# Tony-Tseng/deep-rawburst-sr

Hardware: AMD Instinct MI355X
Metric: bursts/sec 14x48x48 RAW->4x (SyntheticBurstVal shape), DBSR forward (higher is better)
Workload: dtype fp16; 1 GPU; configs[1]: SyntheticBurstVal 14-frame 48x48 -> 384x384 (sr x8 of RAW, x4 of full-res), batch 8 per GPU, full PWC-Net + warp + fusion + decoder; global_batch=8, frames=14, height=48, width=48, out_size=384, parallelism=dp1 (independent bursts per rank), hip_graph=True, fusion_weights_written=True

## Files before the change

deep-rawburst-sr_amd/_lib.py:

```python
import ctypes
import os

import torch

_HERE = os.path.dirname(os.path.abspath(__file__))
LIB_PATH = os.environ.get('DBSR_HIP_LIB', os.path.join(_HERE, 'libdbsr_hip.so'))

DBSR_F32, DBSR_BF16, DBSR_F16 = 0, 1, 2
ACT_NONE, ACT_RELU, ACT_LRELU = 0, 1, 2
OUT_NHWC, OUT_SHUFFLE, OUT_NCHW_F32 = 0, 1, 2
ABI_VERSION = 23
SRC_F32_NCHW, SRC_U8_NHWC = 0, 1
POST_GAINS, POST_CCM, POST_GAMMA, POST_SMOOTHSTEP = 1, 2, 4, 8


class FrameMap(ctypes.Structure):
    _fields_ = [('fpg', ctypes.c_int), ('group_stride', ctypes.c_int), ('group_offset', ctypes.c_int),
                ('inner_stride', ctypes.c_int)]


IDENTITY = (1, 1, 0, 1)


class Tensor(ctypes.Structure):
# ... 39 lines not shown
_lib = None


class DBSRLibError(RuntimeError):
    pass


def lib():
    global _lib
    if _lib is None:
        if not os.path.exists(LIB_PATH):
            raise DBSRLibError('libdbsr_hip.so not found at %s: build it with `make` (or __graft_entry__.build())'
                               % LIB_PATH)
        L = ctypes.CDLL(LIB_PATH)
        c_int, c_void_p, c_float, c_ll, c_size_t = (ctypes.c_int, ctypes.c_void_p, ctypes.c_float,
                                                    ctypes.c_longlong, ctypes.c_size_t)
        sigs = {
            'dbsr_abi_version': ([], c_int),
            'dbsr_last_error': ([], ctypes.c_char_p),
            'dbsr_conv_packed_elems': ([c_int, c_int, c_int, c_int], c_size_t),
            'dbsr_weights_round_diffuse': ([c_void_p, c_int, c_int, c_int, c_int, c_int, c_void_p, c_void_p], c_int),
            'dbsr_conv_pack_weights': ([c_void_p, c_void_p, c_int, c_int, c_int, c_int, c_int, c_int, c_void_p,
                                        c_void_p, c_void_p], c_int),
            'dbsr_pack_batch_prepare': ([ctypes.POINTER(PackJob), c_int], c_ll),
            'dbsr_conv_pack_weights_batch': ([c_void_p, c_int, c_ll, c_void_p], c_int),
            'dbsr_conv2d': ([ctypes.POINTER(ConvDesc), c_void_p], c_int),
            'dbsr_set_conv_algo': ([c_int], c_int),
            'dbsr_conv_kernel_for': ([ctypes.POINTER(ConvDesc)], c_int),
            'dbsr_conv_dispatch_variant': ([ctypes.POINTER(ConvDesc)], c_int),
            'dbsr_conv_lane_reach': ([ctypes.POINTER(ConvDesc), c_int], c_int),
            'dbsr_conv_workspace_bytes': ([ctypes.POINTER(ConvDesc)], c_size_t),
            'dbsr_conv2d_head': ([ctypes.POINTER(ConvDesc), c_void_p, c_void_p, c_int, Tensor, c_void_p], c_int),
            'dbsr_conv_head_ok': ([ctypes.POINTER(ConvDesc)], c_int),
            'dbsr_conv_shuffle_blur': ([ctypes.POINTER(ConvDesc), c_void_p, c_void_p], c_int),
            'dbsr_conv_shuffle_blur_ok': ([ctypes.POINTER(ConvDesc)], c_int),
            'dbsr_resblock': ([ctypes.POINTER(ConvDesc), ctypes.POINTER(ConvDesc), c_void_p], c_int),
            'dbsr_resblock_ok': ([ctypes.POINTER(ConvDesc), ctypes.POINTER(ConvDesc)], c_int),
            'dbsr_resblock_head': ([ctypes.POINTER(ConvDesc), ctypes.POINTER(ConvDesc), c_void_p, c_void_p, c_int, Tensor,
                                    c_void_p], c_int),
            'dbsr_correlation': ([c_int, c_int, c_int, c_int, Tensor, Tensor, Tensor, c_int, c_void_p], c_int),
            'dbsr_correlation_backward': ([c_int, c_int, c_int, c_int, Tensor, Tensor, Tensor, Tensor, c_int, Tensor,
                                           Tensor, c_void_p], c_int),
            'dbsr_backwarp': ([c_int, c_int, c_int, c_int, Tensor, Tensor, c_float, Tensor, c_void_p], c_int),
            'dbsr_warp_bilinear': ([c_int, c_int, c_int, c_int, Tensor, c_void_p, c_ll, Tensor, c_void_p], c_int),
            'dbsr_warp_project': ([c_int, c_int, c_int, c_int, Tensor, c_void_p, c_ll, Tensor, c_void_p, c_void_p, c_int,
                                   Tensor, c_void_p], c_int),
            'dbsr_fuse_relu_norm': ([c_int, c_int, c_int, c_int, Tensor, Tensor, Tensor, Tensor, Tensor, c_void_p], c_int),
            'dbsr_burst_mean': ([c_int, c_int, c_int, c_int, Tensor, Tensor, c_void_p], c_int),
            'dbsr_fuse_softmax': ([c_int, c_int, c_int, c_int, Tensor, Tensor, Tensor, Tensor, Tensor, c_void_p],
                                  c_int),
            'dbsr_conv_fuse_softmax': ([ctypes.POINTER(ConvDesc), c_int, c_int, Tensor, Tensor, Tensor, Tensor,
                                        c_void_p], c_int),
            'dbsr_conv_fuse_relu_norm': ([ctypes.POINTER(ConvDesc), c_int, c_int, Tensor, Tensor, Tensor, Tensor,
                                          c_void_p], c_int),
            'dbsr_conv_fuse_ok': ([ctypes.POINTER(ConvDesc), c_int, c_int], c_int),
            'dbsr_fuse_partial': ([c_int, c_int, c_int, c_int, c_int, Tensor, Tensor, Tensor, c_void_p, c_void_p], c_int),
            'dbsr_fuse_combine': ([c_int, c_int, c_int, c_int, c_void_p, Tensor, c_void_p], c_int),
            'dbsr_conv_transpose_k4s2': ([c_int, c_int, c_int, c_int, c_int, Tensor, c_void_p, c_void_p, Tensor,
                                          c_void_p], c_int),
            'dbsr_pack_burst': ([c_int, c_int, c_int, c_int, c_void_p, Tensor, c_int, c_int, Tensor, c_void_p], c_int),
            'dbsr_flow_finalize': ([c_int, c_int, c_int, c_int, Tensor, c_int, c_int, c_int, c_int, c_void_p, c_float,
                                    Tensor, c_void_p], c_int),
            'dbsr_gauss_blur3': ([c_int, c_int, c_int, c_int, Tensor, c_void_p, Tensor, c_void_p], c_int),
            'dbsr_merge_prep': ([c_int, c_int, c_int, c_int, Tensor, Tensor, c_void_p], c_int),
            'dbsr_pwc_assemble': ([c_int, c_int, c_int, c_int, Tensor, Tensor, Tensor, Tensor, c_void_p], c_int),
            'dbsr_zero': ([c_void_p, c_size_t, c_void_p], c_int),
# ... 56 lines not shown
            'dbsr_burst_synth': ([c_int, c_int, c_int, c_int, c_int, c_int, c_void_p, c_void_p, c_void_p, c_void_p,
                                  c_void_p, c_void_p, c_void_p, c_void_p], c_int),
            'dbsr_postprocess_rgb': ([c_int, c_int, c_int, c_void_p, c_void_p, c_int, c_void_p, c_void_p, c_void_p],
                                     c_int),
        }
        for name, (args, res) in sigs.items():
            fn = getattr(L, name)
            fn.argtypes = args
            fn.restype = res
        if L.dbsr_abi_version() != ABI_VERSION:
            raise DBSRLibError('libdbsr_hip.so ABI %d != expected %d' % (L.dbsr_abi_version(), ABI_VERSION))
        _lib = L
    return _lib


EXPORTED = ['dbsr_abi_version', 'dbsr_last_error', 'dbsr_conv_packed_elems', 'dbsr_conv_pack_weights',
            'dbsr_pack_batch_prepare', 'dbsr_conv_pack_weights_batch',
            'dbsr_weights_round_diffuse', 'dbsr_fuse_relu_norm', 'dbsr_burst_mean', 'dbsr_conv2d',
            'dbsr_set_conv_algo', 'dbsr_conv_kernel_for', 'dbsr_conv_dispatch_variant', 'dbsr_conv_lane_reach', 'dbsr_conv_workspace_bytes', 'dbsr_conv2d_head',
            'dbsr_conv_head_ok', 'dbsr_conv_shuffle_blur', 'dbsr_conv_shuffle_blur_ok', 'dbsr_resblock', 'dbsr_resblock_ok', 'dbsr_resblock_head',
            'dbsr_correlation', 'dbsr_correlation_backward', 'dbsr_backwarp', 'dbsr_warp_bilinear', 'dbsr_warp_project', 'dbsr_fuse_softmax',
            'dbsr_fuse_partial', 'dbsr_fuse_combine', 'dbsr_conv_fuse_softmax', 'dbsr_conv_fuse_relu_norm', 'dbsr_conv_fuse_ok',
            'dbsr_conv_transpose_k4s2', 'dbsr_pack_burst', 'dbsr_flow_finalize', 'dbsr_gauss_blur3',
            'dbsr_merge_prep', 'dbsr_pwc_assemble', 'dbsr_zero', 'dbsr_nhwc_to_nchw_f32', 'dbsr_conv_wgrad_workspace_bytes', 'dbsr_conv_wgrad', 'dbsr_conv_wgrad_bias', 'dbsr_set_wgrad_algo', 'dbsr_head_forward', 'dbsr_head_backward_workspace_bytes', 'dbsr_head_backward',
            'dbsr_chan_sum_workspace_bytes', 'dbsr_chan_sum', 'dbsr_l1_loss_backward', 'dbsr_relu_grad', 'dbsr_unshuffle_gate',
            'dbsr_fuse_backward', 'dbsr_merge_prep_backward', 'dbsr_warp_backward', 'dbsr_enc_grad_gate',
            'dbsr_warp_backward_gather_workspace_bytes', 'dbsr_warp_backward_gather', 'dbsr_gate_copy',
            'dbsr_adam_step', 'dbsr_dgrad_weights',
            'dbsr_resize_bilinear', 'dbsr_gauss_reflect', 'dbsr_color_fit', 'dbsr_color_apply', 'dbsr_pwc_dense',
            'dbsr_pwc_dense_supported', 'dbsr_pwc_refine', 'dbsr_pwc_refine_supported', 'dbsr_pwc_extract',
            'dbsr_pwc_extract_supported', 'dbsr_pwc_level_prep', 'dbsr_pwc_level_prep_supported',
            'dbsr_aligned_l1_workspace_bytes', 'dbsr_aligned_l1_forward', 'dbsr_aligned_l1_backward',
            'dbsr_ssim_workspace_bytes', 'dbsr_ssim_forward', 'dbsr_ssim_backward',
            'dbsr_unprocess_rgb', 'dbsr_burst_synth', 'dbsr_postprocess_rgb']


def check(rc, what):
    if rc != 0:
        msg = lib().dbsr_last_error().decode(errors='replace')
        raise DBSRLibError('%s failed (rc=%d): %s' % (what, rc, msg))


def dtype_code(dt):
    if dt == torch.float32:
        return DBSR_F32
    if dt == torch.bfloat16:
        return DBSR_BF16
    if dt == torch.float16:
        return DBSR_F16
    raise ValueError('unsupported dtype %s' % dt)


def tensor_desc(t, ld, c0=0, img_stride=None, fmap=IDENTITY, dtype=None):
    if t is None:
        return Tensor(None, 0, 0, 0, 0, FrameMap(1, 1, 0, 1))
    if img_stride is None:
        img_stride = t[0].numel() if t.dim() > 1 else t.numel()
    return Tensor(t.data_ptr(), dtype_code(t.dtype if dtype is None else dtype), int(img_stride), int(ld), int(c0),
                  FrameMap(*fmap))


NULL_TENSOR = Tensor(None, 0, 0, 0, 0, FrameMap(1, 1, 0, 1))


def stream_ptr(device=None):
    return torch.cuda.current_stream(device).cuda_stream
```

deep-rawburst-sr_amd/engine.py:

```python
import ctypes
import math
import os
import types

import torch

from . import _lib as L
from ._lib import IDENTITY

BACKWARP_SCALE = {5: 0.625, 4: 1.25, 3: 2.5, 2: 5.0}
PWC_LEVEL_CH = {1: 16, 2: 32, 3: 64, 4: 96, 5: 128, 6: 196}
DENSE_OUT = [128, 128, 96, 64, 32]
DENSE_OFF = [320, 192, 96, 32, 0]
BASE_OFF = 448
REFINER_TAIL = [(128, 128, 3, 2), (128, 128, 3, 4), (128, 96, 3, 8), (96, 64, 3, 16), (64, 32, 3, 1), (32, 2, 3, 1)]


def r8(c):
    return (c + 7) // 8 * 8


def cpad(c):
    return r8(c) if c <= 16 else (c + 31) // 32 * 32

# ... 169 lines not shown
        return st

    def switch(self, lane):
        assert lane == 0 or lane in self.streams or not Plan.MULTI_STREAM
        self.lane = lane if Plan.MULTI_STREAM else 0

    def join(self, lane):
        if not Plan.MULTI_STREAM:
            return
        assert lane != 0 and lane in self.streams
        self.ops.append((Plan.JOIN, (torch.cuda.Event(),), f'sync.join{lane}', lane))
        self.lane = 0

    def conv(self, name, pc, n_frames, x, xc0, in_hw, y, yc0, act, xmap=IDENTITY, ymap=IDENTITY, res=None,
             rc0=0, rmap=IDENTITY, post_act=L.ACT_NONE, out_mode=L.OUT_NHWC, shuffle=0, y_desc=None, cin=None,
             precise=False, head=None, gate=None, gc0=0, gmap=IDENTITY):
        d = self._desc(name, pc, n_frames, x, xc0, in_hw, y, yc0, act, xmap, ymap, res, rc0, rmap, post_act,
                       out_mode, shuffle, y_desc, cin, precise, gate, gc0, gmap)
        self.convs.append((d, self.lane))
        oh, ow = d.out_h, d.out_w
        flop = 2.0 * n_frames * oh * ow * pc.cout * d.cin * pc.kh * pc.kw
        d.fused_head = bool(head is not None and L.lib().dbsr_conv_head_ok(ctypes.byref(d)))
        if d.fused_head:
            hname, hw, hb, hdesc = head
            self.keep.extend([hw, hb, hdesc])
            flop += 2.0 * n_frames * oh * ow * hw.shape[0] * hw.shape[1]
            self.add(name + '+' + hname, L.lib().dbsr_conv2d_head, ctypes.byref(d), hw.data_ptr(),
                     hb.data_ptr() if hb is not None else None, hw.shape[0], hdesc, work=('flop', flop))
            self.kernel[len(self.ops) - 1] = 'conv3x3_pipe'
            return d
        self.add(name, L.lib().dbsr_conv2d, ctypes.byref(d), work=('flop', flop))
        self.kernel[len(self.ops) - 1] = {4: 'conv3x3_ws', 7: 'conv3x3_ks128', 2: 'conv3x3_pipe', 1: 'conv3x3_tiled', 3: 'conv1x1_shuffle', 5: 'conv1x1', 6: 'conv3x3_narrow', 8: 'conv3x3_small'}.get(L.lib().dbsr_conv_kernel_for(d),
                                                                                      'conv2d_generic')
        return d

    def conv_fuse(self, name, pc, B, N, x, in_hw, ref, oth, fused, weights, xmap=IDENTITY, softmax=True):
        d = self._desc(name, pc, B * N, x, 0, in_hw, None, 0, L.ACT_NONE, xmap, IDENTITY, None, 0, IDENTITY,
                       L.ACT_NONE, L.OUT_NHWC, 0, L.NULL_TENSOR, None, False, None, 0, IDENTITY)
        if not L.lib().dbsr_conv_fuse_ok(ctypes.byref(d), B, N):
            return None
        H, W = in_hw
        flop = 2.0 * B * N * H * W * pc.cout * d.cin * pc.kh * pc.kw
        fn = L.lib().dbsr_conv_fuse_softmax if softmax else L.lib().dbsr_conv_fuse_relu_norm
        self.add(name, fn, ctypes.byref(d), B, N, ref, oth, fused, weights,
                 work=('flop', flop))
        self.kernel[len(self.ops) - 1] = 'conv_fuse'
        es, C = (4 if x.dtype == torch.float32 else 2), pc.cout
        self.hbm[len(self.ops) - 1] = es * B * H * W * (N * d.cin + N * C + (N * C if weights.ptr else 0) + C)
        return len(self.ops) - 1

    def resblock(self, name, c1, c2, n_frames, x, mid, y, hw, head=None, yc0=0):
        d1 = self._desc(name + '.conv1', c1, n_frames, x, 0, hw, mid, 0, L.ACT_RELU, IDENTITY, IDENTITY, None, 0,
                        IDENTITY, L.ACT_NONE, L.OUT_NHWC, 0, None, None, False, None, 0, IDENTITY)
        d2 = self._desc(name + '.conv2', c2, n_frames, mid, 0, hw, y, yc0, L.ACT_NONE, IDENTITY, IDENTITY, x, 0,
                        IDENTITY, L.ACT_RELU, L.OUT_NHWC, 0, None, None, False, None, 0, IDENTITY)
        if (c1.cout == 64 and not DBSREngine.FUSED_RESBLOCK64) or \
                not L.lib().dbsr_resblock_ok(ctypes.byref(d1), ctypes.byref(d2)):
            return False
        self.convs.extend([(d1, self.lane), (d2, self.lane)])
        oh, ow = d1.out_h, d1.out_w
        flop = 2.0 * n_frames * oh * ow * (c1.cout * d1.cin * 9 + c2.cout * d2.cin * 9)
        if head is not None:
            hname, hw_, hb, hdesc = head
            self.keep.extend([hw_, hb, hdesc])
            flop += 2.0 * n_frames * oh * ow * hw_.shape[0] * hw_.shape[1]
            self.add(name + '+' + hname, L.lib().dbsr_resblock_head, ctypes.byref(d1), ctypes.byref(d2),
# ... 261 lines not shown
                    plan.add(f'pwc.dec{level}.upflow', lib.dbsr_conv_transpose_k4s2, P, pD.h, pD.w, 2, 2, pflow.d(0),
                             wt.data_ptr(), bs.data_ptr(), fu.d(0))
                    wt, bs = ent['upfeat']
                    plan.add(f'pwc.dec{level}.upfeat', lib.dbsr_conv_transpose_k4s2, P, pD.h, pD.w, BASE_OFF + pbase,
                             2, pD.d(0), wt.data_ptr(), bs.data_ptr(), fe.d(0))
                    ws = NHWC(P, h, w, cpad(C), dtype, device)
                    plan.add(f'pwc.dec{level}.backwarp', lib.dbsr_backwarp, P, h, w, C, feat.d(0, second_map), fu.d(0),
                             BACKWARP_SCALE[level], ws.d(0))
                    plan.add(f'pwc.dec{level}.assemble', lib.dbsr_pwc_assemble, P, h, w, C, feat.d(0, first_map),
                             fu.d(0), fe.d(0), D.d(BASE_OFF))
                    second = ws.d(0)
                    plan.keep.extend([fu, fe, ws])
                plan.add(f'pwc.dec{level}.corr', lib.dbsr_correlation, P, h, w, C, feat.d(0, first_map), second,
                         D.d(BASE_OFF), 1)
            fl = NHWC(P, h, w, 8, torch.float32, device)
            if PWCPlanner.FUSED_DENSE and dtype != torch.float32 and lib.dbsr_pwc_dense_supported(h, w, ld):
                convs = (L.PwcDenseConv * 6)()
                cin, flop = base_real, 0.0
                for i, pc in enumerate(ent['dense'] + [ent['flow']]):
                    start = 0 if i == 5 else (BASE_OFF if i == 0 else DENSE_OFF[i - 1])
                    cg = cpad(pc.cin) // 8
                    convs[i] = L.PwcDenseConv(pc.w.data_ptr(), pc.bias.data_ptr() if pc.bias is not None else None,
                                              9 * cg * 8, cg, start, pc.cout, DENSE_OFF[i] if i < 5 else 0)
                    flop += 2.0 * P * h * w * pc.cout * pc.cin * 9
                plan.keep.append(convs)
                plan.add(f'pwc.dec{level}.dense', lib.dbsr_pwc_dense, P, h, w, D.d(0), BASE_OFF, convs, fl.d(0),
                         work=('flop', flop))
                plan.kernel[len(plan.ops) - 1] = 'pwc_dense'
                cin = base_real + sum(DENSE_OUT)
            else:
                cin = base_real
                for i, (pc, off) in enumerate(zip(ent['dense'], DENSE_OFF)):
                    start = BASE_OFF if i == 0 else DENSE_OFF[i - 1]
                    plan.conv(f'pwc.dec{level}.dense{i}', pc, P, D, start, (h, w), D, off, L.ACT_LRELU, cin=cin)
                    cin += DENSE_OUT[i]
                plan.conv(f'pwc.dec{level}.flow', ent['flow'], P, D, 0, (h, w), None, 0, L.ACT_NONE, cin=cin,
                          y_desc=fl.d(0))
            plan.keep.extend([D, fl])
            prev = (D, fl, base_real)
        D2, fl2, base2 = prev
        h, w = D2.h, D2.w
        chans = [128, 128, 128, 96, 64, 32]
        bufs = [NHWC(P, h, w, cpad(c), dtype, device) for c in chans]
        x, xc0, cin = D2, 0, BASE_OFF + base2
        fused = PWCPlanner.FUSED_REFINER and dtype != torch.float32 and \
            lib.dbsr_pwc_refine_supported(h, w, L.dtype_code(dtype)) and \
            [(pc.cin, pc.cout, pc.kh, pc.dil) for pc in self.ref[1:]] == REFINER_TAIL
        for i in range(1 if fused else 6):
            pc = self.ref[i]
            if pc.dil >= h and pc.dil >= w and pc.kh == 3:
                pc = self.ref_center(i)
            plan.conv(f'pwc.refiner{i}', pc, P, x, xc0, (h, w), bufs[i], 0, L.ACT_LRELU, cin=cin)
            x, xc0, cin = bufs[i], 0, chans[i]
        if fused:
            pcs = [self.ref_center(i) if i == 4 else self.ref[i] for i in range(1, 7)]
            convs = (L.PwcRefineConv * 6)(*[
                L.PwcRefineConv(pc.w.data_ptr(), pc.bias.data_ptr() if pc.bias is not None else None, pc.cin, pc.cout,
                                pc.kh, pc.dil) for pc in pcs])
            flop = sum(2.0 * P * h * w * pc.cout * pc.cin * pc.kh * pc.kw for pc in pcs)
            plan.keep.append(convs)
            plan.add('pwc.refiner1-6', lib.dbsr_pwc_refine, P, h, w, x.d(0), convs, fl2.d(0), flow_out.d(0),
                     work=('flop', flop))
            plan.kernel[len(plan.ops) - 1] = 'pwc_dense'
        else:
            plan.conv('pwc.refiner6', self.ref[6], P, x, 0, (h, w), None, 0, L.ACT_NONE, y_desc=flow_out.d(0),
                      res=fl2)
        plan.keep.extend(bufs)


class DBSREngine:
    LANE0_CU_SHARE = 0.5625
    LANE0_EARLY_CONVS = 0
    LANE0_EARLY_SHARE = 0.5
    FUSED_HEAD = True
    FUSED_UPSAMPLE_BLUR = True
    FUSED_RESBLOCK = True
    FUSED_RESBLOCK64 = True
    FUSED_WARP_PROJ = False
    LINEAR_SPLIT = True
    FUSED_WP_OUT = True
    WEIGHT_ROUNDING = 'diffuse'

    def __init__(self, net):
        self.net = net
        self.dtype = net.compute_dtype
        self.zero_flow = bool(getattr(net, 'zero_flow', False))
        self.device = None
        self.sig = None
        self.plans = {}
        self.slots = {}
        self.graphs = {}
        self.weights_stale = False

    def matches(self, net):
        return (net is self.net and self.dtype == net.compute_dtype and self.sig == _param_signature(net)
                and self.zero_flow == bool(getattr(net, 'zero_flow', False)))

    def _pack(self, device):
        net = self.net
        stream = L.stream_ptr(device)
        W = _Weights(self.dtype, device, stream, rounding=DBSREngine.WEIGHT_ROUNDING)
        enc, mer, dec = net.encoder, net.merging, net.decoder
        self.pwc = PWCPlanner(enc.alignment_net, _Weights(self.dtype, device, stream))
        self.enc_init = W.conv(enc.init_layer[0])
        self.enc_res = [(W.conv(b.conv1[0]), W.conv(b.conv2[0])) for b in enc.res_layers]
        self.enc_out = W.conv(enc.out_layer[0])
        self.proj = W.conv(mer.feat_project_layer[0])
        ofe = list(mer.offset_feat_extractor)
        self.ofe_init = W.conv(ofe[0][0])
        self.ofe_res = [(W.conv(b.conv1[0]), W.conv(b.conv2[0])) for b in ofe[1:]]
        wp = list(mer.weight_predictor)
        self.wp_init = W.conv(wp[0][0])
        self.softmax, self.ref_base, self.offset_modulo = merging_variant(mer)
        pd = mer.feat_project_layer[0].out_channels
# ... 218 lines not shown
        rgb = NHWC(F, Hp, Wp, 8, dt, dev)
        bufs['offsets'] = torch.zeros(P, 2, H, W, dtype=torch.float32, device=dev)
        om = NHWC(F, H, W, 8, dt, dev)
        E = NHWC(F, H, W, C, dt, dev)
        PJ = NHWC(F, H, W, r8(self.proj.cout), dt, dev) if self.wp_split is None else None
        sh = {'rgb': rgb, 'offsets': bufs['offsets'], 'om': om, 'E': E, 'PJ': PJ, 'Hp': Hp, 'Wp': Wp}
        grp = (0, B)
        plan.add('pack_burst', lib.dbsr_pack_burst, B, N, H, W, bufs['burst'].data_ptr(), raw.d(0), Hp, Wp,
                 rgb.d(0) if not self.zero_flow else L.NULL_TENSOR)
        plan_cap = int(torch.cuda.get_device_properties(dev).multi_processor_count * DBSREngine.LANE0_CU_SHARE) \
            if Plan.MULTI_STREAM else 0
        plan.fork(1, dev, priority=0)
        WP = self._emit_flow(plan, grp, N, H, W, sh)
        plan.switch(0)
        plan.max_blocks = plan.max_blocks_cap = plan_cap
        if plan_cap and DBSREngine.LANE0_EARLY_CONVS:
            names = ['enc.init'] + [f'enc.res{i}.conv{j}' for i in range(len(self.enc_res)) for j in (1, 2)]
            plan.early_names = set(names[:DBSREngine.LANE0_EARLY_CONVS])
            plan.early_cap = int(torch.cuda.get_device_properties(dev).multi_processor_count *
                                 DBSREngine.LANE0_EARLY_SHARE)
        e = [NHWC(F, H, W, r8(self.enc_init.cout), dt, dev) for _ in range(3)]
        plan.conv('enc.init', self.enc_init, F, raw, 0, hw, e[0], 0, L.ACT_RELU)
        i = self._resblocks(plan, 'enc.res', self.enc_res, F, hw, e, 0, dt)
        plan.conv('enc.out', self.enc_out, F, e[i], 0, hw, E, 0, L.ACT_RELU)
        if self.wp_split is None:
            plan.conv('merge.proj_ref', self.proj, B, E, 0, hw, PJ, 0, L.ACT_RELU, xmap=(1, N, 0, 1),
                      ymap=(1, N, 0, 1))
        plan.keep.extend([raw, rgb, om, e, E, PJ])
        FW = NHWC(F, H, W, C, dt, dev) if mode == 'full' else None
        if mode == 'full':
            bufs['pred'] = torch.zeros(B, 3, H * self.s, W * self.s, dtype=torch.float32, device=dev)
        plan.fuse_ops = []
        es = 4 if dt == torch.float32 else 2
        BS = self._emit_base(plan, grp, N, H, W, sh, WP) if self.wp_split is not None else None
        plan.join(1)
        plan.max_blocks = 0
        plan.switch(1)
        self._emit_ofe(plan, grp, N, H, W, sh, WP)
        plan.switch(0)
        Wf = self._emit_warp(plan, grp, N, H, W, sh, WP)
        plan.join(1)
        h, Wf = self._emit_merge(plan, grp, N, H, W, sh, WP, BS=BS, Wf=Wf)
        if mode == 'partial':
            LG = self._emit_logits(plan, B * N, H, W, h)
            ST = torch.zeros(B, H, W, 3 * C, dtype=torch.float32, device=dev)
            plan.add('merge.fuse_partial', lib.dbsr_fuse_partial, B, N, H * W, C, first_frame, LG.d(0),
                     E.d(0, (1, N, 0, 1)), Wf.d(0), ST.data_ptr())
            bufs['stats'] = ST
        else:
            FUS = NHWC(B, H, W, C, dt, dev)
            feats = [E.d(0, (1, N, 0, 1)), Wf.d(0), FUS.d(0), FW.d(0)]
            idx = plan.conv_fuse('merge.wp.out+fuse', self.wp_out, B, N, h, hw, *feats, softmax=self.softmax) \
                if DBSREngine.FUSED_WP_OUT else None
            if idx is not None:
                plan.fuse_ops.append((idx, plan.ops[idx][1], FW.d(0), None))
            else:
                LG = self._emit_logits(plan, B * N, H, W, h)
                args = [B, N, H * W, C, LG.d(0)] + feats
                if self.softmax:
                    plan.add('merge.fuse', lib.dbsr_fuse_softmax, *args)
                else:
                    plan.add('merge.fuse_relu_norm', lib.dbsr_fuse_relu_norm, *args)
                plan.fuse_ops.append((len(plan.ops) - 1, args, FW.d(0),
                                      ((2.0 * N + 1) * B * C * H * W * es, 1.0 * N * B * C * H * W * es)))
            self._decoder(plan, B, H, W, FUS, bufs, pred_out=bufs['pred'])
            plan.keep.append(FUS)
        plan.max_blocks = 0
        plan.keep.append(FW)
        plan.finalize_workspace(dev)
        plan.bufs = bufs
        plan.FW = FW
        plan.shape = (B, N, H, W)
        return plan

    def _decoder(self, plan, B, H, W, FUS, bufs, pred_out=None):
        dt, dev = self.dtype, self.device
        lib = L.lib()
        hw = (H, W)
        S = self.s
        gd = self.dec_init.cout
        g = [NHWC(B, H, W, gd, dt, dev) for _ in range(3)]
        plan.conv('dec.init', self.dec_init, B, FUS, 0, hw, g[0], 0, L.ACT_RELU)
        i = self._resblocks(plan, 'dec.pre', self.dec_pre, B, hw, g, 0, dt)
        pc = self.dec_up.cout // (S * S)
        sh = [NHWC(B, H * S, W * S, pc, dt, dev) for _ in range(3)]
        a = 0
        if self.blur is not None and DBSREngine.FUSED_UPSAMPLE_BLUR and \
                plan.conv_shuffle_blur('dec.upsample+blur', self.dec_up, B, g[i], hw, sh[1], L.ACT_RELU,
                                       self.blur) is not None:
            a = 1
        else:
            plan.conv('dec.upsample', self.dec_up, B, g[i], 0, hw, sh[0], 0, L.ACT_RELU, out_mode=L.OUT_SHUFFLE,
                      shuffle=S)
            if self.blur is not None:
                kbuf = (ctypes.c_float * 9)(*self.blur)
                plan.keep.append(kbuf)
                plan.add('dec.blur', lib.dbsr_gauss_blur3, B, H * S, W * S, pc, sh[0].d(0), kbuf, sh[1].d(0))
                a = 1
        if pred_out is None:
            pred_out = bufs['pred'] = torch.zeros(B, 3, H * S, W * S, dtype=torch.float32, device=dev)
        pdesc = L.tensor_desc(pred_out, 1, 0, img_stride=3 * H * S * W * S, dtype=torch.float32)
        head = None
        if dt != torch.float32 and self.dec_post and DBSREngine.FUSED_HEAD:
            head = ('predictor', self.head_w, self.head_b, pdesc)
        if head is not None:
            i, fused = self._resblocks(plan, 'dec.post', self.dec_post, B, (H * S, W * S), sh, a, dt, head=head)
        else:
            i, fused = self._resblocks(plan, 'dec.post', self.dec_post, B, (H * S, W * S), sh, a, dt), False
        if not fused:
            plan.conv('dec.predictor', self.pred, B, sh[i], 0, (H * S, W * S), None, 0, L.ACT_RELU,
                      out_mode=L.OUT_NCHW_F32, y_desc=pdesc, precise=(dt != torch.float32))
        plan.keep.extend([g, sh])

    @staticmethod
    def _capture(plan, dev):
# ... 213 lines not shown
```

deep-rawburst-sr_amd/ops.py:

```python
import collections

import torch

from . import _lib as L


def _nhwc(x, dtype=None):
    t = x.permute(0, 2, 3, 1)
    if dtype is not None:
        t = t.to(dtype)
    c = t.shape[-1]
    ld = (c + 7) // 8 * 8 if c <= 16 else (c + 31) // 32 * 32
    out = torch.zeros(*t.shape[:-1], ld, dtype=t.dtype, device=t.device)
    out[..., :c] = t
    return out, ld


def _need_cuda(*ts):
    for t in ts:
        if not t.is_cuda:
            raise NotImplementedError('dbsr_amd ops run on the HIP device only (no CPU implementation, as '
                                      'correlation.py:324-325)')


# ... 90 lines not shown
    d.in_h, d.in_w, d.cin = H, W, Cin
    d.w = wp.data_ptr()
    d.bias = bp.data_ptr() if bp is not None else None
    d.cout, d.kh, d.kw, d.stride, d.pad, d.dil = Cout, kh, kw, stride, padding, dilation
    d.y = L.tensor_desc(y, ldy)
    d.out_h, d.out_w = oh, ow
    d.act = act
    if residual is not None:
        rr, ldr = _nhwc(residual, ody)
        d.res = L.tensor_desc(rr, ldr)
    else:
        d.res = L.NULL_TENSOR
    d.post_act = post_act
    d.out_mode, d.shuffle = (L.OUT_SHUFFLE, shuffle) if shuffle > 1 else (L.OUT_NHWC, 0)
    need = L.lib().dbsr_conv_workspace_bytes(d)
    ws = torch.zeros(max(need // 4, 1), dtype=torch.float32, device=dev)
    d.workspace, d.workspace_bytes = ws.data_ptr(), need
    if head is not None:
        hw, hb = head
        hc = hw.shape[0]
        hw32 = hw.reshape(hc, -1).to(device=dev, dtype=torch.float32).contiguous()
        hb32 = hb.to(device=dev, dtype=torch.float32).contiguous() if hb is not None else None
        out = torch.zeros(N, hc, oh, ow, dtype=torch.float32, device=dev)
        L.check(L.lib().dbsr_conv2d_head(d, hw32.data_ptr(), hb32.data_ptr() if hb32 is not None else None, hc,
                                         L.tensor_desc(out, 1, 0, img_stride=hc * oh * ow, dtype=torch.float32),
                                         s), 'dbsr_conv2d_head')
        return out
    conv2d.last_kernel = L.lib().dbsr_conv_kernel_for(d)
    conv2d.last_variant = L.lib().dbsr_conv_dispatch_variant(d)
    L.check(L.lib().dbsr_conv2d(d, s), 'dbsr_conv2d')
    return y[..., :pc].permute(0, 3, 1, 2).contiguous()


def conv2d_wgrad(x, dy, k, compute_dtype=torch.float32, with_bias=False):
    _need_cuda(x, dy)
    N, Cin, H, W = x.shape
    Cout = dy.shape[1]
    xs, ldx = _nhwc(x, compute_dtype)
    ds, ldd = _nhwc(dy, compute_dtype)
    dw = torch.zeros(Cout, Cin, k, k, dtype=torch.float32, device=x.device)
    need = L.lib().dbsr_conv_wgrad_workspace_bytes(N, H, W, Cin, Cout, k)
    ws = torch.empty(max(need // 4, 1), dtype=torch.float32, device=x.device)
    if not with_bias:
        L.check(L.lib().dbsr_conv_wgrad(N, H, W, L.tensor_desc(xs, ldx), Cin, L.tensor_desc(ds, ldd), Cout, k,
                                        dw.data_ptr(), 0, ws.data_ptr(), need, L.stream_ptr(x.device)),
                'dbsr_conv_wgrad')
        return dw
    db = torch.zeros(Cout, dtype=torch.float32, device=x.device)
    L.check(L.lib().dbsr_conv_wgrad_bias(N, H, W, L.tensor_desc(xs, ldx), Cin, L.tensor_desc(ds, ldd), Cout, k,
                                         dw.data_ptr(), db.data_ptr(), 0, ws.data_ptr(), need,
                                         L.stream_ptr(x.device)), 'dbsr_conv_wgrad_bias')
    return dw, db


def conv2d_dgrad(dy, weight, residual=None, gate=None, compute_dtype=torch.float32):
    _need_cuda(dy, weight)
    Cout, Cin, kh, kw = weight.shape
    w32 = weight.to(torch.float32).contiguous()
    wt = torch.empty(Cin, Cout, kh, kw, dtype=torch.float32, device=dy.device)
    s = L.stream_ptr(dy.device)
    L.check(L.lib().dbsr_dgrad_weights(w32.data_ptr(), Cout, Cin, kh, kw, wt.data_ptr(), s), 'dbsr_dgrad_weights')
    N, _, H, W = dy.shape
    ds, ldd = _nhwc(dy, compute_dtype)
    n = L.lib().dbsr_conv_packed_elems(Cin, Cout, kh, kw)
    wp = torch.empty(n, dtype=compute_dtype, device=dy.device)
    L.check(L.lib().dbsr_conv_pack_weights(wt.data_ptr(), None, Cin, Cout, kh, kw, L.dtype_code(compute_dtype), 1,
# ... 267 lines not shown
```

include/dbsr_hip.h:

```cpp
#ifndef DBSR_HIP_H
#define DBSR_HIP_H

#include <stddef.h>
#include <stdint.h>

#ifdef __cplusplus
extern "C" {
#endif

#define DBSR_ABI_VERSION 23

enum { DBSR_F32 = 0, DBSR_BF16 = 1, DBSR_F16 = 2 };
enum { DBSR_ACT_NONE = 0, DBSR_ACT_RELU = 1, DBSR_ACT_LRELU = 2 };
enum { DBSR_OUT_NHWC = 0, DBSR_OUT_SHUFFLE = 1, DBSR_OUT_NCHW_F32 = 2 };
enum { DBSR_E_ARG = -1, DBSR_E_UNSUPPORTED = -2 };

typedef struct dbsr_frame_map {
    int fpg;
    int group_stride;
    int group_offset;
    int inner_stride;
} dbsr_frame_map;

typedef struct dbsr_tensor {
// ... 24 lines not shown

size_t dbsr_conv_packed_elems(int cout, int cin, int kh, int kw);
int dbsr_conv_pack_weights(const float* w_f32, const float* bias_f32, int cout, int cin, int kh, int kw,
                           int dtype, int shuffle, void* w_packed, float* bias_out, void* stream);
typedef struct dbsr_pack_job {
    const float* w;
    const float* bias;
    void* w_packed;
    float* bias_out;
    int cout, cin, kh, kw;
    int dtype, shuffle;
    int transposed, lo, src_cin;
    int pad_;
    long long blk0;
} dbsr_pack_job;
long long dbsr_pack_batch_prepare(dbsr_pack_job* jobs, int n);
int dbsr_conv_pack_weights_batch(const dbsr_pack_job* jobs_dev, int n, long long n_blocks, void* stream);
int dbsr_conv2d(const dbsr_conv_desc* d, void* stream);
int dbsr_weights_round_diffuse(const float* w, int cout, int cin, int kh, int kw, int dtype, float* w_out,
                               void* stream);
int dbsr_set_conv_algo(int algo);
int dbsr_conv_kernel_for(const dbsr_conv_desc* d);
int dbsr_conv_dispatch_variant(const dbsr_conv_desc* d);
int dbsr_conv_lane_reach(const dbsr_conv_desc* d, int which);
int dbsr_conv2d_head(const dbsr_conv_desc* d, const float* head_w, const float* head_b, int head_cout,
                     dbsr_tensor head_out, void* stream);
int dbsr_conv_shuffle_blur(const dbsr_conv_desc* d, const float* k9, void* stream);
int dbsr_conv_shuffle_blur_ok(const dbsr_conv_desc* d);
int dbsr_resblock(const dbsr_conv_desc* c1, const dbsr_conv_desc* c2, void* stream);
int dbsr_resblock_ok(const dbsr_conv_desc* c1, const dbsr_conv_desc* c2);
int dbsr_resblock_head(const dbsr_conv_desc* c1, const dbsr_conv_desc* c2, const float* head_w, const float* head_b,
                       int head_cout, dbsr_tensor head_out, void* stream);
int dbsr_conv_head_ok(const dbsr_conv_desc* d);
size_t dbsr_conv_workspace_bytes(const dbsr_conv_desc* d);

int dbsr_correlation(int n_pairs, int h, int w, int c, dbsr_tensor first, dbsr_tensor second,
                     dbsr_tensor out, int leaky, void* stream);

int dbsr_correlation_backward(int n_pairs, int h, int w, int c, dbsr_tensor first, dbsr_tensor second,
                              dbsr_tensor out, dbsr_tensor gout, int leaky, dbsr_tensor dfirst, dbsr_tensor dsecond,
                              void* stream);

int dbsr_backwarp(int n, int h, int w, int c, dbsr_tensor in, dbsr_tensor flow, float scale,
                  dbsr_tensor out, void* stream);

int dbsr_warp_bilinear(int n, int h, int w, int c, dbsr_tensor feat, const float* flow,
                       long long flow_img_stride, dbsr_tensor out, void* stream);
int dbsr_warp_project(int n, int h, int w, int c, dbsr_tensor feat, const float* flow, long long flow_img_stride,
                      dbsr_tensor out, const void* proj_w, const float* proj_b, int proj_cout, dbsr_tensor proj_out,
                      void* stream);

int dbsr_fuse_softmax(int B, int N, int hw, int c, dbsr_tensor logits, dbsr_tensor ref, dbsr_tensor oth,
                      dbsr_tensor fused, dbsr_tensor weights, void* stream);

int dbsr_fuse_relu_norm(int B, int N, int hw, int c, dbsr_tensor logits, dbsr_tensor ref, dbsr_tensor oth,
                        dbsr_tensor fused, dbsr_tensor weights, void* stream);
int dbsr_burst_mean(int B, int N, int hw, int c, dbsr_tensor in, dbsr_tensor out, void* stream);

int dbsr_conv_fuse_softmax(const dbsr_conv_desc* d, int B, int N, dbsr_tensor ref, dbsr_tensor oth,
                           dbsr_tensor fused, dbsr_tensor weights, void* stream);
int dbsr_conv_fuse_relu_norm(const dbsr_conv_desc* d, int B, int N, dbsr_tensor ref, dbsr_tensor oth,
                             dbsr_tensor fused, dbsr_tensor weights, void* stream);
int dbsr_conv_fuse_ok(const dbsr_conv_desc* d, int B, int N);

int dbsr_fuse_partial(int B, int N, int hw, int c, int first_frame, dbsr_tensor logits, dbsr_tensor ref,
                      dbsr_tensor oth, float* stats, void* stream);
// ... 138 lines not shown
```

Measured before the change: 3446 bursts/s.

## Add split-K 3x3 conv kernel for narrow-output, deep-input convs

Adds a new MFMA 3x3 conv kernel that splits the input-channel reduction across four waves per block, each with its own double-buffered LDS halo staging, then reduces the partial sums through shared memory before applying bias and activation. It is used for PWC dense-decoder convs with cout 32/64 and for the decoder init conv, where few output channels and many input channels leave the existing kernels with little parallelism per tile. A cost model chooses between two tile shapes. It also adds an optional, off-by-default path that runs the base branch on the side stream next to the optical-flow encoder. The risks are extra LDS reduction traffic and lower occupancy from the large per-block shared memory.

```diff
diff --git a/deep-rawburst-sr_amd/_lib.py b/deep-rawburst-sr_amd/_lib.py
--- a/deep-rawburst-sr_amd/_lib.py
+++ b/deep-rawburst-sr_amd/_lib.py
@@ -95,6 +95,9 @@
             'dbsr_conv_workspace_bytes': ([ctypes.POINTER(ConvDesc)], c_size_t),
             'dbsr_conv2d_head': ([ctypes.POINTER(ConvDesc), c_void_p, c_void_p, c_int, Tensor, c_void_p], c_int),
             'dbsr_conv_head_ok': ([ctypes.POINTER(ConvDesc)], c_int),
+            'dbsr_conv3x3_ksplit': ([ctypes.POINTER(ConvDesc), c_void_p], c_int),
+            'dbsr_conv3x3_ksplit_supported': ([ctypes.POINTER(ConvDesc)], c_int),
+            'dbsr_set_ksplit_tile': ([c_int], c_int),
             'dbsr_conv_shuffle_blur': ([ctypes.POINTER(ConvDesc), c_void_p, c_void_p], c_int),
             'dbsr_conv_shuffle_blur_ok': ([ctypes.POINTER(ConvDesc)], c_int),
             'dbsr_resblock': ([ctypes.POINTER(ConvDesc), ctypes.POINTER(ConvDesc), c_void_p], c_int),
@@ -217,7 +220,8 @@
             'dbsr_pwc_extract_supported', 'dbsr_pwc_level_prep', 'dbsr_pwc_level_prep_supported',
             'dbsr_aligned_l1_workspace_bytes', 'dbsr_aligned_l1_forward', 'dbsr_aligned_l1_backward',
             'dbsr_ssim_workspace_bytes', 'dbsr_ssim_forward', 'dbsr_ssim_backward',
-            'dbsr_unprocess_rgb', 'dbsr_burst_synth', 'dbsr_postprocess_rgb']
+            'dbsr_unprocess_rgb', 'dbsr_burst_synth', 'dbsr_postprocess_rgb',
+            'dbsr_conv3x3_ksplit', 'dbsr_conv3x3_ksplit_supported', 'dbsr_set_ksplit_tile']
 
 
 def check(rc, what):
diff --git a/deep-rawburst-sr_amd/csrc/conv_ksplit.hip b/deep-rawburst-sr_amd/csrc/conv_ksplit.hip
--- /dev/null
+++ b/deep-rawburst-sr_amd/csrc/conv_ksplit.hip
@@ -0,0 +1,304 @@
+#include "conv_core.hpp"
+
+#include <type_traits>
+
+using namespace dbsr;
+
+namespace {
+
+typedef __attribute__((ext_vector_type(8))) __bf16 bfv8_t;
+typedef __attribute__((ext_vector_type(8))) _Float16 hv8_t;
+
+template <typename T>
+__device__ __forceinline__ f32x4_t ks_mma(u32x4_t a, u32x4_t b, f32x4_t c) {
+    if constexpr (std::is_same<T, bf16_t>::value)
+        return __builtin_amdgcn_mfma_f32_16x16x32_bf16(__builtin_bit_cast(bfv8_t, a), __builtin_bit_cast(bfv8_t, b), c,
+                                                       0, 0, 0);
+    else
+        return __builtin_amdgcn_mfma_f32_16x16x32_f16(__builtin_bit_cast(hv8_t, a), __builtin_bit_cast(hv8_t, b), c,
+                                                      0, 0, 0);
+}
+
+constexpr int KS_WAVES = 4;
+__host__ __device__ constexpr int ks_hp(int nt) { return nt == 8 ? 12 : 7; }
+
+struct KsArgs {
+    dbsr_tensor x, y;
+    const void* w_pipe;
+    const float* bias;
+    int h, w, cin, nch, act;
+    int tw, th, tiles_x, tiles_y;
+};
+
+template <typename T, int NT, int MB>
+__global__ __launch_bounds__(256) void conv3x3_ksplit_kernel(KsArgs a) {
+    constexpr int HP = ks_hp(NT);
+    constexpr int BUF = HP * 512;
+    constexpr int PPT = (HP + 5) / 6;
+    constexpr int AD = MB == 4 ? 3 : 9;
+    constexpr int STG_BYTES = KS_WAVES * 2 * BUF * 2;
+    constexpr int RED_BYTES = KS_WAVES * NT * MB * 64 * 16;
+    __shared__ __attribute__((aligned(16))) u32x4_t smem[(STG_BYTES > RED_BYTES ? STG_BYTES : RED_BYTES) / 16];
+
+    const int lane = threadIdx.x & 63, wave = __builtin_amdgcn_readfirstlane(threadIdx.x >> 6);
+    const int g = lane >> 4, col = lane & 15;
+    int bid = blockIdx.x;
+    const int tx = bid % a.tiles_x;
+    bid /= a.tiles_x;
+    const int ty = bid % a.tiles_y, f = bid / a.tiles_y;
+    const int x0 = tx * a.tw, y0 = ty * a.th;
+    const int hw_ = a.tw + 2, nhp = hw_ * (a.th + 2);
+    const T* xf = img_ptr<const T>(a.x, f);
+
+    const int q8 = (lane & 3) * 8;
+    int poff[HP];
+    unsigned inside = 0;
+#pragma unroll
+    for (int i = 0; i < HP; ++i) {
+        const int hp = 16 * i + (lane >> 2);
+        const int hy = hp / hw_, hx = hp - hy * hw_;
+        const int gy = y0 - 1 + hy, gx = x0 - 1 + hx;
+        const bool ok = hp < nhp && gy >= 0 && gy < a.h && gx >= 0 && gx < a.w;
+        poff[i] = ok ? (gy * a.w + gx) * a.x.ld : 0;
+        inside |= ok ? 1u << i : 0u;
+    }
+    int bbase[NT];
+#pragma unroll
+    for (int t = 0; t < NT; ++t) {
+        const int p = 16 * t + col;
+        const int py = p / a.tw, px = p - py * a.tw;
+        bbase[t] = (p < a.tw * a.th ? (py * hw_ + px) * 32 : 0) + g * 8;
+    }
+    const int c_lo = wave * a.nch / KS_WAVES, c_hi = (wave + 1) * a.nch / KS_WAVES;
+    const int cin8 = (a.cin + 7) & ~7;
+    const T* wl = (const T*)a.w_pipe + lane * 8;
+    T* cur = (T*)smem + wave * 2 * BUF;
+    T* nxt = cur + BUF;
+
+    auto stage_load = [&](int c, int i) {
+        return *(const u32x4_t*)(xf + poff[i] + min(c * 32 + q8, cin8 - 8));
+    };
+    auto stage_mask = [&](int c, int i, u32x4_t v) {
+        const int keep = min(max(a.cin - (c * 32 + q8), 0), 8);
+        const bool ok = (inside >> i) & 1u;
+#pragma unroll
+        for (int d = 0; d < 4; ++d) {
+            const unsigned m = keep >= 2 * d + 2 ? 0xffffffffu : keep == 2 * d + 1 ? 0x0000ffffu : 0u;
+            v[d] = ok ? v[d] & m : 0u;
+        }
+        return v;
+    };
+    const long long wm = (long long)a.nch * 9 * 512;
+    auto weight_at = [&](int m, int c, int tap) {
+        return *(const u32x4_t*)(wl + m * wm + (long long)(c * 9 + tap) * 512);
+    };
+    auto lds_order = [&]() {
+        __builtin_amdgcn_fence(__ATOMIC_ACQ_REL, "wavefront");
+        __builtin_amdgcn_wave_barrier();
+    };
+
+    f32x4_t acc[NT][MB];
+#pragma unroll
+    for (int t = 0; t < NT; ++t)
+#pragma unroll
+        for (int m = 0; m < MB; ++m) acc[t][m] = f32x4_t{0.f, 0.f, 0.f, 0.f};
+
+    u32x4_t A[AD][MB];
+#pragma unroll
+    for (int tap = 0; tap < AD; ++tap)
+#pragma unroll
+        for (int m = 0; m < MB; ++m) A[tap][m] = weight_at(m, c_lo, tap);
+#pragma unroll
+    for (int i = 0; i < HP; ++i) *(u32x4_t*)(cur + i * 512 + lane * 8) = stage_mask(c_lo, i, stage_load(c_lo, i));
+    u32x4_t Bq[2][NT];
+    lds_order();
+#pragma unroll
+    for (int t = 0; t < NT; ++t) Bq[0][t] = *(const u32x4_t*)(cur + bbase[t]);
+
+    u32x4_t S[3][PPT];
+    auto chunk = [&](int c, auto has_next_c) {
+        constexpr bool has_next = decltype(has_next_c)::value;
+        StaticFor<0, 9>::run([&](auto tap_c) {
+            constexpr int tap = decltype(tap_c)::value;
+            if constexpr (has_next && tap >= 3) {
+#pragma unroll
+                for (int k = 0; k < PPT; ++k)
+                    if ((tap - 3) * PPT + k < HP)
+                        *(u32x4_t*)(nxt + ((tap - 3) * PPT + k) * 512 + lane * 8) =
+                            stage_mask(c + 1, (tap - 3) * PPT + k, S[tap % 3][k]);
+            }
+            if constexpr (tap < 8) {
+                const int toff = (((tap + 1) / 3) * hw_ + (tap + 1) % 3) * 32;
+#pragma unroll
+                for (int t = 0; t < NT; ++t) Bq[(tap + 1) & 1][t] = *(const u32x4_t*)(cur + bbase[t] + toff);
+            }
+            __builtin_amdgcn_sched_barrier(0);
+#pragma unroll
+            for (int t = 0; t < NT; ++t)
+#pragma unroll
+                for (int m = 0; m < MB; ++m) acc[t][m] = ks_mma<T>(A[tap % AD][m], Bq[tap & 1][t], acc[t][m]);
+            if constexpr (tap + AD < 9) {
+#pragma unroll
+                for (int m = 0; m < MB; ++m) A[tap % AD][m] = weight_at(m, c, tap + AD);
+            } else if constexpr (has_next) {
+#pragma unroll
+                for (int m = 0; m < MB; ++m) A[tap % AD][m] = weight_at(m, c + 1, tap + AD - 9);
+            }
+            if constexpr (has_next) {
+                if constexpr (tap < 6) {
+#pragma unroll
+                    for (int k = 0; k < PPT; ++k)
+                        if (tap * PPT + k < HP) S[tap % 3][k] = stage_load(c + 1, tap * PPT + k);
+                }
+                if constexpr (tap == 8) {
+                    lds_order();
+#pragma unroll
+                    for (int t = 0; t < NT; ++t) Bq[0][t] = *(const u32x4_t*)(nxt + bbase[t]);
+                }
+            }
+            __builtin_amdgcn_sched_barrier(0);
+        });
+        T* t_ = cur;
+        cur = nxt;
+        nxt = t_;
+    };
+    for (int c = c_lo; c + 1 < c_hi; ++c) chunk(c, std::true_type{});
+    chunk(c_hi - 1, std::false_type{});
+
+    __syncthreads();
+    f32x4_t* red = (f32x4_t*)smem;
+#pragma unroll
+    for (int t = 0; t < NT; ++t)
+#pragma unroll
+        for (int m = 0; m < MB; ++m) red[((wave * NT + t) * MB + m) * 64 + lane] = acc[t][m];
+    __syncthreads();
+    T* yf = img_ptr<T>(a.y, f);
+    for (int t = wave; t < NT; t += KS_WAVES) {
+        const int p = 16 * t + col;
+        const int py = p / a.tw, px = p - py * a.tw;
+        const int oy = y0 + py, ox = x0 + px;
+        const bool ok = p < a.tw * a.th && oy < a.h && ox < a.w;
+#pragma unroll
+        for (int j = 0; j < MB / 2; ++j) {
+            float v[8];
+#pragma unroll
+            for (int hm = 0; hm < 2; ++hm) {
+                f32x4_t s = red[((0 * NT + t) * MB + 2 * j + hm) * 64 + lane];
+#pragma unroll
+                for (int wv = 1; wv < KS_WAVES; ++wv) s += red[((wv * NT + t) * MB + 2 * j + hm) * 64 + lane];
+#pragma unroll
+                for (int r = 0; r < 4; ++r) v[4 * hm + r] = s[r];
+            }
+            const int co = 32 * j + 8 * g;
+            if (a.bias) {
+#pragma unroll
+                for (int r = 0; r < 8; ++r) v[r] += a.bias[co + r];
+            }
+#pragma unroll
+            for (int r = 0; r < 8; ++r) v[r] = apply_act(v[r], a.act);
+            if (ok) store8(yf + (long long)(oy * a.w + ox) * a.y.ld + co, v);
+        }
+    }
+}
+
+int ks_num_cus() {
+    static int cus = 0;
+    if (!cus) {
+        int dev = 0;
+        (void)hipGetDevice(&dev);
+        (void)hipDeviceGetAttribute(&cus, hipDeviceAttributeMultiprocessorCount, dev);
+        if (cus <= 0) cus = 256;
+    }
+    return cus;
+}
+
+const char* ks_refusal(const dbsr_conv_desc* d) {
+    if (!d) return "null desc";
+    if (!d->x.ptr || !d->y.ptr || !d->w || d->x.map.fpg <= 0 || d->y.map.fpg <= 0) return "null tensor";
+    if (!is16(d->x.dtype) || d->y.dtype != d->x.dtype || d->precise) return "x and y must both be bf16 or both fp16";
+    if (d->kh != 3 || d->kw != 3 || d->stride != 1 || d->pad != 1 || d->dil != 1)
+        return "needs a 3x3 conv with stride 1, pad 1, dilation 1";
+    if (d->cout != 32 && d->cout != 64) return "cout must be 32 or 64";
+    if (d->cin <= 0 || cin_pad(d->cin) < 256) return "cin (padded to 32) must be at least 256";
+    if (d->n_frames <= 0 || d->in_h <= 0 || d->in_w <= 0 || d->out_h != d->in_h || d->out_w != d->in_w)
+        return "inconsistent geometry";
+    if (d->act != DBSR_ACT_NONE && d->act != DBSR_ACT_RELU && d->act != DBSR_ACT_LRELU) return "unknown activation";
+    if (d->res.ptr || d->gate.ptr || d->post_act != DBSR_ACT_NONE || d->out_mode != DBSR_OUT_NHWC || d->shuffle > 1)
+        return "no residual, gate, post-activation, shuffle or NCHW output";
+    if (d->x.ld % 8 || d->x.c0 % 8 || d->y.ld % 8 || d->y.c0 % 8 || d->x.c0 < 0 || d->y.c0 < 0)
+        return "ld and c0 must be multiples of 8";
+    if (d->x.c0 + round_up(d->cin, 8) > d->x.ld) return "input slice c0 + cin exceeds ld";
+    if (d->y.c0 + d->cout > d->y.ld) return "output slice c0 + cout exceeds ld";
+    if ((long long)d->in_h * d->in_w * d->x.ld >= (1ll << 31) || (long long)d->in_h * d->in_w * d->y.ld >= (1ll << 31))
+        return "frame too large";
+    if (d->x.ptr == d->y.ptr && d->x.c0 < d->y.c0 + d->cout && d->y.c0 < d->x.c0 + round_up(d->cin, 8))
+        return "output channels overlap the input slice";
+    return nullptr;
+}
+
+struct KsTile { int nt, tw, th; };
+int g_ks_tile = 0;
+KsTile ks_tile(const dbsr_conv_desc* d, int cus) {
+    const KsTile cand[2] = {{8, 16, 8}, {5, 12, 6}};
+    const int cinp = cin_pad(d->cin), mb = d->cout / 16;
+    if (g_ks_tile == 8) return cand[0];
+    if (g_ks_tile == 5) return cand[1];
+    KsTile best = cand[0];
+    double best_cost = 0.;
+    for (int i = 0; i < 2; ++i) {
+        const KsTile& k = cand[i];
+        const long long blocks = (long long)d->n_frames * ((d->in_w + k.tw - 1) / k.tw) * ((d->in_h + k.th - 1) / k.th);
+        const double rounds = (double)((blocks + cus - 1) / cus);
+        const double bytes = 2.0 * cinp * (9.0 * d->cout + (k.tw + 2) * (k.th + 2));
+        const double mfma = 16.0 * k.nt * mb * 9 * (cinp / 32) / 4;
+        const double cost = rounds * (bytes / 32 > mfma ? bytes / 32 : mfma);
+        if (i == 0 || cost < best_cost) {
+            best = k;
+            best_cost = cost;
+        }
+    }
+    return best;
+}
+
+}
+
+extern "C" int dbsr_set_ksplit_tile(int nt) {
+    DBSR_CHECK_ARG(nt == 0 || nt == 8 || nt == 5, "set_ksplit_tile: 0 (by cost), 8 (16 x 8) or 5 (12 x 6)");
+    g_ks_tile = nt;
+    return 0;
+}
+
+extern "C" int dbsr_conv3x3_ksplit_supported(const dbsr_conv_desc* d) { return ks_refusal(d) ? 0 : 1; }
+
+extern "C" int dbsr_conv3x3_ksplit(const dbsr_conv_desc* d, void* stream) {
+    const char* why = ks_refusal(d);
+    DBSR_CHECK_ARG(!why, "conv3x3_ksplit: %s", why);
+    const KsTile tile = ks_tile(d, ks_num_cus());
+    const int cinp = cin_pad(d->cin);
+    KsArgs a;
+    a.x = d->x;
+    a.y = d->y;
+    a.w_pipe = (const char*)d->w + (size_t)round_up(d->cout, 64) * 9 * cinp * 2;
+    a.bias = d->bias;
+    a.h = d->in_h; a.w = d->in_w; a.cin = d->cin; a.nch = cinp / 32; a.act = d->act;
+    a.tw = tile.tw; a.th = tile.th;
+    a.tiles_x = (d->in_w + tile.tw - 1) / tile.tw;
+    a.tiles_y = (d->in_h + tile.th - 1) / tile.th;
+    const long long blocks = (long long)d->n_frames * a.tiles_x * a.tiles_y;
+    DBSR_CHECK_ARG(blocks < (1ll << 31), "conv3x3_ksplit: too many tiles");
+    hipStream_t s = (hipStream_t)stream;
+    const bool bf = d->x.dtype == DBSR_BF16;
+#define DBSR_KS(NT, MB)                                                                                      \
+    do {                                                                                                     \
+        if (bf) hipLaunchKernelGGL((conv3x3_ksplit_kernel<bf16_t, NT, MB>), dim3((unsigned)blocks), dim3(256), 0, s, a); \
+        else hipLaunchKernelGGL((conv3x3_ksplit_kernel<f16_t, NT, MB>), dim3((unsigned)blocks), dim3(256), 0, s, a);     \
+    } while (0)
+    if (tile.nt == 8) {
+        if (d->cout == 64) DBSR_KS(8, 4); else DBSR_KS(8, 2);
+    } else {
+        if (d->cout == 64) DBSR_KS(5, 4); else DBSR_KS(5, 2);
+    }
+#undef DBSR_KS
+    DBSR_LAUNCH_CHECK();
+    return 0;
+}
diff --git a/deep-rawburst-sr_amd/engine.py b/deep-rawburst-sr_amd/engine.py
--- a/deep-rawburst-sr_amd/engine.py
+++ b/deep-rawburst-sr_amd/engine.py
@@ -225,6 +225,20 @@
         self.add(name, L.lib().dbsr_conv2d, ctypes.byref(d), work=('flop', flop))
         self.kernel[len(self.ops) - 1] = {4: 'conv3x3_ws', 7: 'conv3x3_ks128', 2: 'conv3x3_pipe', 1: 'conv3x3_tiled', 3: 'conv1x1_shuffle', 5: 'conv1x1', 6: 'conv3x3_narrow', 8: 'conv3x3_small'}.get(L.lib().dbsr_conv_kernel_for(d),
                                                                                       'conv2d_generic')
+        return d
+
+    def conv_ksplit(self, name, pc, n_frames, x, xc0, in_hw, y, yc0, act, cin=None):
+        if not DBSREngine.KSPLIT_CONV:
+            return None
+        keep = len(self.keep)
+        d = self._desc(name, pc, n_frames, x, xc0, in_hw, y, yc0, act, IDENTITY, IDENTITY, None, 0, IDENTITY,
+                       L.ACT_NONE, L.OUT_NHWC, 0, None, cin, False, None, 0, IDENTITY)
+        if not L.lib().dbsr_conv3x3_ksplit_supported(ctypes.byref(d)):
+            del self.keep[keep:]
+            return None
+        flop = 2.0 * n_frames * d.out_h * d.out_w * pc.cout * d.cin * pc.kh * pc.kw
+        self.add(name, L.lib().dbsr_conv3x3_ksplit, ctypes.byref(d), work=('flop', flop))
+        self.kernel[len(self.ops) - 1] = 'conv3x3_tiled'
         return d
 
     def conv_fuse(self, name, pc, B, N, x, in_hw, ref, oth, fused, weights, xmap=IDENTITY, softmax=True):
@@ -552,7 +566,9 @@
                 cin = base_real
                 for i, (pc, off) in enumerate(zip(ent['dense'], DENSE_OFF)):
                     start = BASE_OFF if i == 0 else DENSE_OFF[i - 1]
-                    plan.conv(f'pwc.dec{level}.dense{i}', pc, P, D, start, (h, w), D, off, L.ACT_LRELU, cin=cin)
+                    if pc.cout > 64 or plan.conv_ksplit(f'pwc.dec{level}.dense{i}', pc, P, D, start, (h, w), D, off,
+                                                        L.ACT_LRELU, cin=cin) is None:
+                        plan.conv(f'pwc.dec{level}.dense{i}', pc, P, D, start, (h, w), D, off, L.ACT_LRELU, cin=cin)
                     cin += DENSE_OUT[i]
                 plan.conv(f'pwc.dec{level}.flow', ent['flow'], P, D, 0, (h, w), None, 0, L.ACT_NONE, cin=cin,
                           y_desc=fl.d(0))
@@ -600,6 +616,8 @@
     LINEAR_SPLIT = True
     FUSED_WP_OUT = True
     WEIGHT_ROUNDING = 'diffuse'
+    KSPLIT_CONV = os.environ.get('DBSR_KSPLIT_CONV', '1') != '0'
+    BASE_BESIDE_WARP = os.environ.get('DBSR_BASE_BESIDE_WARP', '0') == '1'
 
     def __init__(self, net):
         self.net = net
@@ -884,11 +902,19 @@
             bufs['pred'] = torch.zeros(B, 3, H * self.s, W * self.s, dtype=torch.float32, device=dev)
         plan.fuse_ops = []
         es = 4 if dt == torch.float32 else 2
-        BS = self._emit_base(plan, grp, N, H, W, sh, WP) if self.wp_split is not None else None
+        beside = DBSREngine.BASE_BESIDE_WARP and Plan.MULTI_STREAM and self.wp_split is not None
+        BS = None
+        if self.wp_split is not None and not beside:
+            BS = self._emit_base(plan, grp, N, H, W, sh, WP)
         plan.join(1)
         plan.max_blocks = 0
-        plan.switch(1)
+        if beside:
+            plan.fork(1, dev, priority=0)
+        else:
+            plan.switch(1)
         self._emit_ofe(plan, grp, N, H, W, sh, WP)
+        if beside:
+            BS = self._emit_base(plan, grp, N, H, W, sh, WP)
         plan.switch(0)
         Wf = self._emit_warp(plan, grp, N, H, W, sh, WP)
         plan.join(1)
@@ -932,7 +958,8 @@
         S = self.s
         gd = self.dec_init.cout
         g = [NHWC(B, H, W, gd, dt, dev) for _ in range(3)]
-        plan.conv('dec.init', self.dec_init, B, FUS, 0, hw, g[0], 0, L.ACT_RELU)
+        if plan.conv_ksplit('dec.init', self.dec_init, B, FUS, 0, hw, g[0], 0, L.ACT_RELU) is None:
+            plan.conv('dec.init', self.dec_init, B, FUS, 0, hw, g[0], 0, L.ACT_RELU)
         i = self._resblocks(plan, 'dec.pre', self.dec_pre, B, hw, g, 0, dt)
         pc = self.dec_up.cout // (S * S)
         sh = [NHWC(B, H * S, W * S, pc, dt, dev) for _ in range(3)]
diff --git a/deep-rawburst-sr_amd/ops.py b/deep-rawburst-sr_amd/ops.py
--- a/deep-rawburst-sr_amd/ops.py
+++ b/deep-rawburst-sr_amd/ops.py
@@ -146,6 +146,32 @@
     return y[..., :pc].permute(0, 3, 1, 2).contiguous()
 
 
+def conv3x3_ksplit(x, weight, bias=None, act=L.ACT_NONE, compute_dtype=torch.float16):
+    _need_cuda(x, weight)
+    N, Cin, H, W = x.shape
+    Cout = weight.shape[0]
+    dev = x.device
+    xs, ldx = _nhwc(x, compute_dtype)
+    s = L.stream_ptr(dev)
+    wp, bp = _packed(weight, bias, compute_dtype, 1, s)
+    ldy = (Cout + 7) // 8 * 8
+    y = torch.zeros(N, H, W, ldy, dtype=compute_dtype, device=dev)
+    d = L.ConvDesc()
+    d.n_frames = N
+    d.x = L.tensor_desc(xs, ldx)
+    d.in_h, d.in_w, d.cin = H, W, Cin
+    d.w = wp.data_ptr()
+    d.bias = bp.data_ptr() if bp is not None else None
+    d.cout, d.kh, d.kw, d.stride, d.pad, d.dil = Cout, weight.shape[2], weight.shape[3], 1, 1, 1
+    d.y = L.tensor_desc(y, ldy)
+    d.out_h, d.out_w = H, W
+    d.act = act
+    d.res = d.gate = L.NULL_TENSOR
+    d.out_mode = L.OUT_NHWC
+    L.check(L.lib().dbsr_conv3x3_ksplit(d, s), 'dbsr_conv3x3_ksplit')
+    return y[..., :Cout].permute(0, 3, 1, 2).contiguous()
+
+
 def conv2d_wgrad(x, dy, k, compute_dtype=torch.float32, with_bias=False):
     _need_cuda(x, dy)
     N, Cin, H, W = x.shape
diff --git a/include/dbsr_hip.h b/include/dbsr_hip.h
--- a/include/dbsr_hip.h
+++ b/include/dbsr_hip.h
@@ -80,6 +80,9 @@
 int dbsr_resblock_head(const dbsr_conv_desc* c1, const dbsr_conv_desc* c2, const float* head_w, const float* head_b,
                        int head_cout, dbsr_tensor head_out, void* stream);
 int dbsr_conv_head_ok(const dbsr_conv_desc* d);
+int dbsr_conv3x3_ksplit(const dbsr_conv_desc* d, void* stream);
+int dbsr_conv3x3_ksplit_supported(const dbsr_conv_desc* d);
+int dbsr_set_ksplit_tile(int nt);
 size_t dbsr_conv_workspace_bytes(const dbsr_conv_desc* d);
 
 int dbsr_correlation(int n_pairs, int h, int w, int c, dbsr_tensor first, dbsr_tensor second,
```

New measurement: 3475 bursts/s (median of 6 runs). Within noise of the previous version (+0.8%).
